# deepinv/deepinv

Measured on AMD Instinct MI355X. Metric: PnP-PGD slices/sec (50 iters), 2D MRI 8-coil 320x320, 4x radial mask, DRUNet, higher is better.
Workload: dtype f32: fp32 multiplies and accumulation on the fp32 matrix cores (v_mfma_f32_32x32x2_f32); ResBlock convs as Winograd F(4x4,3x3), U = G g G^T formed in fp64 and rounded once; the three 2x2 stride-2 down convolutions (2 % of the FLOPs) as an exact three-part bf16 operand split with six products and fp3

## Files before the change

### deepinv_amd/csrc/drunet_bf16s.hip

```cpp
#include "drunet_common.hpp"

using namespace dinv;
using namespace dinv_drunet;

namespace {

__device__ __forceinline__ unsigned f2bf(float f) {
#ifdef DINV_EMU
    unsigned u = __float_as_uint(f);
    if ((u & 0x7fffffffu) > 0x7f800000u) return (u >> 16) | 0x40u;
    u += 0x7fffu + ((u >> 16) & 1u);
    return u >> 16;
#else
    return (unsigned)__builtin_bit_cast(unsigned short, (__bf16)f);
#endif
}
__device__ __forceinline__ float bf2f(unsigned h) { return __uint_as_float(h << 16); }

__device__ __forceinline__ void split8(const float4& a, const float4& b, uint4& hi, uint4& lo) {
    const float v[8] = {a.x, a.y, a.z, a.w, b.x, b.y, b.z, b.w};
    unsigned h[8], l[8];
#pragma unroll
    for (int e = 0; e < 8; ++e) {
        h[e] = f2bf(v[e]);
        l[e] = f2bf(v[e] - bf2f(h[e]));
    }
    hi = make_uint4(h[0] | (h[1] << 16), h[2] | (h[3] << 16), h[4] | (h[5] << 16), h[6] | (h[7] << 16));
    lo = make_uint4(l[0] | (l[1] << 16), l[2] | (l[3] << 16), l[4] | (l[5] << 16), l[6] | (l[7] << 16));
}

__device__ __forceinline__ void split8x3(const float4& a, const float4& b, uint4& hi, uint4& mi, uint4& lo) {
    const float v[8] = {a.x, a.y, a.z, a.w, b.x, b.y, b.z, b.w};
    unsigned h[8], m[8], l[8];
#pragma unroll
    for (int e = 0; e < 8; ++e) {
        h[e] = f2bf(v[e]);
        const float r1 = v[e] - bf2f(h[e]);
        m[e] = f2bf(r1);
        l[e] = f2bf(r1 - bf2f(m[e]));
    }
    hi = make_uint4(h[0] | (h[1] << 16), h[2] | (h[3] << 16), h[4] | (h[5] << 16), h[6] | (h[7] << 16));
    mi = make_uint4(m[0] | (m[1] << 16), m[2] | (m[3] << 16), m[4] | (m[5] << 16), m[6] | (m[7] << 16));
    lo = make_uint4(l[0] | (l[1] << 16), l[2] | (l[3] << 16), l[4] | (l[5] << 16), l[6] | (l[7] << 16));
}

#ifdef DINV_EMU
__device__ __forceinline__ f32x16 mfma_bf16(const uint4& a, const uint4& b, const f32x16& c) {
    emu_bf16x8 av, bv;
    std::memcpy(&av, &a, 16);
    std::memcpy(&bv, &b, 16);
    return emu_mfma_f32_32x32x16_bf16(av, bv, c);
}
#else
typedef __bf16 bf16x8 __attribute__((ext_vector_type(8)));
__device__ __forceinline__ f32x16 mfma_bf16(const uint4& a, const uint4& b, const f32x16& c) {
    return __builtin_amdgcn_mfma_f32_32x32x16_bf16(__builtin_bit_cast(bf16x8, a), __builtin_bit_cast(bf16x8, b), c, 0, 0, 0);
}
#endif

struct DownSArgs {
    Geom gi, go;
    const float* x;
    const uint4* w;
    float* y;
    int32_t cin, cout;
    int64_t ntiles, per_xcd;
    DepthMap dm;
};

template <bool ACC, int NPL>
__global__ __launch_bounds__(256) void down2x2_bf16s_kernel(DownSArgs a) {
    constexpr int WU = NPL * 128;
    constexpr int WPT = (WU + 255) / 256;
    __shared__ uint4 wl[2][WU];
    const int tid = threadIdx.x, lane = tid & 63, wv = tid >> 6;
    const int l31 = lane & 31, lhi = lane >> 5;
    const int64_t logical = (int64_t)(blockIdx.x & 7) * a.per_xcd + (blockIdx.x >> 3);
    if (logical >= a.ntiles) return;
    const int nct = a.cout / 64;
    const int64_t q0 = (logical / nct) * 256 + wv * 64;
    const int co0 = (int)(logical % nct) * 64;
    int64_t ioff[2];
    bool in[2];
#pragma unroll
    for (int n = 0; n < 2; ++n) {
        const int64_t q = q0 + n * 32 + l31;
        in[n] = interior(a.go, q);
        ioff[n] = a.gi.sl;
        if (in[n]) {
            const int64_t b = q / a.go.plane;
            const int64_t bi = depth_pair(a.dm, b);
            if (bi < 0) in[n] = false;
            else {
                const int qi = (int)(q - b * a.go.plane);
                const int R = qi / a.go.wp, C = qi - R * a.go.wp;
                ioff[n] = a.gi.sl + bi * a.gi.plane + (int64_t)(2 * (R - 1) + 1) * a.gi.wp + (2 * (C - 1) + 1);
            }
        }
    }
    f32x16 acc[2][2];
#pragma unroll
    for (int m = 0; m < 2; ++m)
#pragma unroll
        for (int n = 0; n < 2; ++n)
#pragma unroll
            for (int r = 0; r < 16; ++r) acc[m][n][r] = 0.f;
    const int S = a.cin / 16, nsteps = 4 * S;
    float4 ba[2], bb[2];
    uint4 wreg[WPT];
    auto issue = [&](int g) {
        const int tap = g / S, s = g - tap * S;
        const int64_t toff = (int64_t)(tap >> 1) * a.gi.wp + (tap & 1);
#pragma unroll
        for (int k = 0; k < WPT; ++k) {
            const int u = tid + 256 * k;
            if (u < WU) wreg[k] = a.w[((int64_t)g * (2 * NPL) + (u >> 6)) * a.cout + co0 + (u & 63)];
        }
#pragma unroll
        for (int n = 0; n < 2; ++n) {
            const float* xb = a.x + ((int64_t)(2 * s + lhi) * a.gi.cs + ioff[n] + toff) * 8;
            ba[n] = ld4(xb);
            bb[n] = ld4(xb + 4);
        }
    };
    uint4 Bp[NPL][2];
    auto commit = [&](int stage) {
#pragma unroll
        for (int k = 0; k < WPT; ++k)
            if (tid + 256 * k < WU) wl[stage][tid + 256 * k] = wreg[k];
#pragma unroll
        for (int n = 0; n < 2; ++n) {
            if constexpr (NPL == 2) split8(ba[n], bb[n], Bp[0][n], Bp[1][n]);
            else split8x3(ba[n], bb[n], Bp[0][n], Bp[1][n], Bp[2][n]);
        }
    };
    issue(0);
    commit(0);
    if (nsteps > 1) issue(1);
    __syncthreads();
    constexpr int NPROD = NPL == 2 ? 3 : 6;
    constexpr int PA[6] = {0, 1, 0, 0, 1, 0}, PB2[3] = {1, 0, 0};
    constexpr int QA[6] = {1, 0, 2, 0, 1, 0}, QB[6] = {1, 2, 0, 1, 0, 0};
    for (int g = 0; g < nsteps; ++g) {
        const uint4* ws = wl[g & 1];
        uint4 A[NPL][2];
#pragma unroll
        for (int pl = 0; pl < NPL; ++pl)
#pragma unroll
            for (int m = 0; m < 2; ++m) A[pl][m] = ws[pl * 128 + lhi * 64 + m * 32 + l31];
#pragma unroll
        for (int e = 0; e < NPROD; ++e) {
            const int pa = NPL == 2 ? PA[e] : QA[e], pb = NPL == 2 ? PB2[e] : QB[e];
#pragma unroll
            for (int m = 0; m < 2; ++m)
#pragma unroll
                for (int n = 0; n < 2; ++n) acc[m][n] = mfma_bf16(A[pa][m], Bp[pb][n], acc[m][n]);
        }
        if (g + 1 < nsteps) {
            commit((g + 1) & 1);
            if (g + 2 < nsteps) issue(g + 2);
        }
        lds_barrier();
    }
#pragma unroll
    for (int n = 0; n < 2; ++n) {
        const int64_t q = q0 + n * 32 + l31;
        if (q >= a.go.np) continue;
        store_tile<2, false, ACC ? 1 : 0>(acc, n, a.go.sl + q, in[n], co0 / 8, a.cout / 8, a.go.cs, lhi, a.y, ACC ? a.y : nullptr,
                                          nullptr);
    }
}

struct UpSArgs {
    Geom gi, go;
    const float* x;
    const float* x2;
    const uint4* w;
    float* y;
    int32_t cin, cout;
    DepthMap dm;
};

#ifdef DINV_EMU
#define DINV_BF16S_UP_ATTR
#else
#define DINV_BF16S_UP_ATTR __attribute__((amdgpu_waves_per_eu(2, 2)))
#endif
template <bool SKIP>
__global__ __launch_bounds__(256) DINV_BF16S_UP_ATTR void up2x2_bf16s_kernel(UpSArgs a) {
    __shared__ uint4 wl[2][1024];
    const int tid = threadIdx.x, lane = tid & 63, wv = tid >> 6;
    const int l31 = lane & 31, lhi = lane >> 5;
    const int tp = wv & 1, pg = wv >> 1;
    const int co0 = blockIdx.y * 64;
    const int64_t p0 = (int64_t)blockIdx.x * 128 + pg * 64;
    int64_t ioff[2], ooff[2];
    bool in[2];
#pragma unroll
    for (int n = 0; n < 2; ++n) {
        const int64_t p = p0 + n * 32 + l31;
        in[n] = interior(a.gi, p);
        ioff[n] = a.gi.sl + (in[n] ? p : 0);
        ooff[n] = 0;
        if (in[n]) {
            const int64_t b = p / a.gi.plane;
            const int64_t bo = depth_pair(a.dm, b);
            if (bo < 0) in[n] = false;
            else {
                const int pi = (int)(p - b * a.gi.plane);
                const int r = pi / a.gi.wp, c = pi - r * a.gi.wp;
                ooff[n] = a.go.sl + bo * a.go.plane + (int64_t)(2 * (r - 1) + 1 + tp) * a.go.wp + (2 * (c - 1) + 1);
            }
        }
    }
    f32x16 acc[2][2][2];
#pragma unroll
    for (int t = 0; t < 2; ++t)
#pragma unroll
        for (int m = 0; m < 2; ++m)
#pragma unroll
            for (int n = 0; n < 2; ++n)
#pragma unroll
                for (int r = 0; r < 16; ++r) acc[t][m][n][r] = 0.f;
    const int S = a.cin / 16;
    float4 ba[2], bb[2];
    uint4 wreg[4];
    auto issue = [&](int s) {
#pragma unroll
        for (int k = 0; k < 4; ++k) {
            const int u = tid + 256 * k;
            wreg[k] = a.w[((int64_t)s * 16 + (u >> 6)) * a.cout + co0 + (u & 63)];
        }
#pragma unroll
        for (int n = 0; n < 2; ++n) {
            const int64_t o = ((int64_t)(2 * s + lhi) * a.gi.cs + ioff[n]) * 8;
            ba[n] = ld4(a.x + o);
            bb[n] = ld4(a.x + o + 4);
            if (SKIP) {
                ba[n] = add4(ba[n], ld4(a.x2 + o));
                bb[n] = add4(bb[n], ld4(a.x2 + o + 4));
            }
        }
    };
    auto commit = [&](int stage, uint4 (&Bh)[2], uint4 (&Bl)[2]) {
#pragma unroll
        for (int k = 0; k < 4; ++k) wl[stage][tid + 256 * k] = wreg[k];
        split8(ba[0], bb[0], Bh[0], Bl[0]);
        split8(ba[1], bb[1], Bh[1], Bl[1]);
    };
    uint4 Bh[2], Bl[2];
    issue(0);
    commit(0, Bh, Bl);
    if (S > 1) issue(1);
    __syncthreads();
    for (int s = 0; s < S; ++s) {
        const uint4* ws = wl[s & 1] + (tp * 2) * 256;
#pragma unroll
        for (int t = 0; t < 2; ++t) {
            uint4 A[2][2];
#pragma unroll
            for (int pl = 0; pl < 2; ++pl)
#pragma unroll
                for (int m = 0; m < 2; ++m) A[pl][m] = ws[t * 256 + pl * 128 + lhi * 64 + m * 32 + l31];
#pragma unroll
            for (int e = 0; e < 3; ++e) {
                const int pa = e == 1 ? 1 : 0;
#pragma unroll
                for (int m = 0; m < 2; ++m)
#pragma unroll
                    for (int n = 0; n < 2; ++n) acc[t][m][n] = mfma_bf16(A[pa][m], e == 0 ? Bl[n] : Bh[n], acc[t][m][n]);
            }
        }
        if (s + 1 < S) {
            commit((s + 1) & 1, Bh, Bl);
            if (s + 2 < S) issue(s + 2);
        }
        lds_barrier();
    }
#pragma unroll
    for (int n = 0; n < 2; ++n) {
        if (!in[n]) continue;
#pragma unroll
        for (int t = 0; t < 2; ++t)
#pragma unroll
            for (int m = 0; m < 2; ++m)
#pragma unroll
                for (int rj = 0; rj < 4; ++rj) {
                    const float4 v = make_float4(acc[t][m][n][4 * rj], acc[t][m][n][4 * rj + 1], acc[t][m][n][4 * rj + 2],
                                                 acc[t][m][n][4 * rj + 3]);
                    st4(a.y + ((int64_t)(co0 / 8 + m * 4 + rj) * a.go.cs + ooff[n] + t) * 8 + 4 * lhi, v);
                }
    }
}

}

static int down2x2_bf16s_launch(const dinv_act_geom* gin, const dinv_act_geom* gout, const float* x, const void* w_split,
                                int32_t cin, int32_t cout, float* y, DepthMap dm, int accumulate, dinv_stream_t stream,
                                int planes = 2) {
    if (int e = check_geom(gin)) return e;
    if (int e = check_geom(gout)) return e;
    DINV_REQUIRE(x && w_split && y, "null tensor pointer");
    DINV_REQUIRE(gin->height == 2 * gout->height && gin->width == 2 * gout->width, "down2x2 geometry mismatch");
    if (dm.dep_s == 0) DINV_REQUIRE(gin->batch == gout->batch, "down2x2 geometry mismatch");
    else
        DINV_REQUIRE(dm.dep_s >= 3 && dm.dep_l == 2 * (dm.dep_s - 2) + 2 && gout->batch % dm.dep_s == 0 &&
                     gin->batch / dm.dep_l == gout->batch / dm.dep_s && gin->batch % dm.dep_l == 0 && (dm.dz == 0 || dm.dz == 1),
                     "down2x2: bad depth pairing (%d, %d, %d)", dm.dep_s, dm.dep_l, dm.dz);
    DINV_REQUIRE(cin >= 16 && cin % 16 == 0 && cout % 64 == 0, "bf16-split down2x2 needs cin %% 16 == 0 and cout %% 64 == 0 (got %d,%d)", cin, cout);
    DownSArgs a{make_geom(*gin), make_geom(*gout), x, reinterpret_cast<const uint4*>(w_split), y, cin, cout, 0, 0, dm};
    a.ntiles = ceil_div(gout->np, 256) * (cout / 64);
    a.per_xcd = ceil_div(a.ntiles, 8);
    const dim3 grid((unsigned)(a.per_xcd * 8));
    hipStream_t st = reinterpret_cast<hipStream_t>(stream);
    if (planes == 3) hipLaunchKernelGGL((down2x2_bf16s_kernel<false, 3>), grid, dim3(256), 0, st, a);
    else if (accumulate) hipLaunchKernelGGL((down2x2_bf16s_kernel<true, 2>), grid, dim3(256), 0, st, a);
    else hipLaunchKernelGGL((down2x2_bf16s_kernel<false, 2>), grid, dim3(256), 0, st, a);
    DINV_CHECK_LAUNCH();
    return 0;
}

extern "C" int dinv_conv_down2x2_bf16s(const dinv_act_geom* gin, const dinv_act_geom* gout, const float* x,
                                       const void* w_split, int32_t cin, int32_t cout, float* y, dinv_stream_t stream) {
    return down2x2_bf16s_launch(gin, gout, x, w_split, cin, cout, y, DepthMap{0, 0, 0}, 0, stream);
}

extern "C" int dinv_conv_down2x2_bf16x3(const dinv_act_geom* gin, const dinv_act_geom* gout, const float* x,
                                        const void* w_split3, int32_t cin, int32_t cout, float* y, dinv_stream_t stream) {
    return down2x2_bf16s_launch(gin, gout, x, w_split3, cin, cout, y, DepthMap{0, 0, 0}, 0, stream, 3);
}

extern "C" int dinv_conv_down2x2_bf16s_3d(const dinv_act_geom* gin, const dinv_act_geom* gout, const float* x,
                                          const void* w_split, int32_t cin, int32_t cout, float* y, int32_t depth_out,
                                          int32_t dz, int32_t accumulate, dinv_stream_t stream) {
    DINV_REQUIRE(depth_out >= 1, "bad depth %d", depth_out);
    return down2x2_bf16s_launch(gin, gout, x, w_split, cin, cout, y, DepthMap{depth_out + 2, 2 * depth_out + 2, dz}, accumulate, stream);
}

static int up2x2_bf16s_launch(const dinv_act_geom* gin, const dinv_act_geom* gout, const float* x, const float* x2,
                              const void* w_split, int32_t cin, int32_t cout, float* y, DepthMap dm, dinv_stream_t stream) {
    if (int e = check_geom(gin)) return e;
    if (int e = check_geom(gout)) return e;
    DINV_REQUIRE(x && w_split && y, "null tensor pointer");
    DINV_REQUIRE(gout->height == 2 * gin->height && gout->width == 2 * gin->width, "up2x2 geometry mismatch");
    if (dm.dep_s == 0) DINV_REQUIRE(gin->batch == gout->batch, "up2x2 geometry mismatch");
    else
        DINV_REQUIRE(dm.dep_s >= 3 && dm.dep_l == 2 * (dm.dep_s - 2) + 2 && gin->batch % dm.dep_s == 0 &&
                     gout->batch % dm.dep_l == 0 && gout->batch / dm.dep_l == gin->batch / dm.dep_s && (dm.dz == 0 || dm.dz == 1),
                     "up2x2: bad depth pairing (%d, %d, %d)", dm.dep_s, dm.dep_l, dm.dz);
    DINV_REQUIRE(cin >= 16 && cin % 16 == 0 && cout % 64 == 0, "bf16-split up2x2 needs cin %% 16 == 0 and cout %% 64 == 0 (got %d,%d)", cin, cout);
    UpSArgs a{make_geom(*gin), make_geom(*gout), x, x2, reinterpret_cast<const uint4*>(w_split), y, cin, cout, dm};
    const dim3 grid((unsigned)ceil_div(gin->np, 128), (unsigned)(cout / 64));
    hipStream_t st = reinterpret_cast<hipStream_t>(stream);
    if (x2) hipLaunchKernelGGL(up2x2_bf16s_kernel<true>, grid, dim3(256), 0, st, a);
    else hipLaunchKernelGGL(up2x2_bf16s_kernel<false>, grid, dim3(256), 0, st, a);
    DINV_CHECK_LAUNCH();
    return 0;
}

extern "C" int dinv_conv_up2x2_bf16s(const dinv_act_geom* gin, const dinv_act_geom* gout, const float* x, const float* x2,
                                     const void* w_split, int32_t cin, int32_t cout, float* y, dinv_stream_t stream) {
    return up2x2_bf16s_launch(gin, gout, x, x2, w_split, cin, cout, y, DepthMap{0, 0, 0}, stream);
}

extern "C" int dinv_conv_up2x2_bf16s_3d(const dinv_act_geom* gin, const dinv_act_geom* gout, const float* x, const float* x2,
                                        const void* w_split, int32_t cin, int32_t cout, float* y, int32_t depth_in, int32_t dz,
                                        dinv_stream_t stream) {
    DINV_REQUIRE(depth_in >= 1, "bad depth %d", depth_in);
    return up2x2_bf16s_launch(gin, gout, x, x2, w_split, cin, cout, y, DepthMap{depth_in + 2, 2 * depth_in + 2, dz}, stream);
}
```

Before: 16.24.

## Deepen down2x2 bf16-split prefetch and add wide 128-channel output tile

Reworks the stride-2 down convolution kernel so each step keeps four register stages of weight and activation loads in flight, with the main loop unrolled by four. This hides global-load latency behind the MFMA work. Separately, it adds a wider tile variant covering 128 output channels per block, used only when enough tiles exist, so each activation split is reused across more MFMAs. The deeper prefetch costs more registers and issues redundant clamped loads near the end of the loop, and the wide path lowers the block count.

```diff
diff --git a/deepinv_amd/csrc/drunet_bf16s.hip b/deepinv_amd/csrc/drunet_bf16s.hip
--- a/deepinv_amd/csrc/drunet_bf16s.hip
+++ b/deepinv_amd/csrc/drunet_bf16s.hip
@@ -68,18 +68,20 @@
     DepthMap dm;
 };
 
-template <bool ACC, int NPL>
+template <bool ACC, int NPL, int MT>
 __global__ __launch_bounds__(256) void down2x2_bf16s_kernel(DownSArgs a) {
-    constexpr int WU = NPL * 128;
+    constexpr int CT = 32 * MT;
+    constexpr int WU = NPL * 2 * CT;
     constexpr int WPT = (WU + 255) / 256;
-    __shared__ uint4 wl[2][WU];
+    constexpr int PF = 4;
+    __shared__ uint4 wl[2][WPT * 256];
     const int tid = threadIdx.x, lane = tid & 63, wv = tid >> 6;
     const int l31 = lane & 31, lhi = lane >> 5;
     const int64_t logical = (int64_t)(blockIdx.x & 7) * a.per_xcd + (blockIdx.x >> 3);
     if (logical >= a.ntiles) return;
-    const int nct = a.cout / 64;
+    const int nct = a.cout / CT;
     const int64_t q0 = (logical / nct) * 256 + wv * 64;
-    const int co0 = (int)(logical % nct) * 64;
+    const int co0 = (int)(logical % nct) * CT;
     int64_t ioff[2];
     bool in[2];
 #pragma unroll
@@ -98,75 +100,85 @@
             }
         }
     }
-    f32x16 acc[2][2];
-#pragma unroll
-    for (int m = 0; m < 2; ++m)
+    f32x16 acc[MT][2];
+#pragma unroll
+    for (int m = 0; m < MT; ++m)
 #pragma unroll
         for (int n = 0; n < 2; ++n)
 #pragma unroll
             for (int r = 0; r < 16; ++r) acc[m][n][r] = 0.f;
     const int S = a.cin / 16, nsteps = 4 * S;
-    float4 ba[2], bb[2];
-    uint4 wreg[WPT];
-    auto issue = [&](int g) {
+    struct Raw {
+        float4 ba[2], bb[2];
+        uint4 w[WPT];
+    };
+    auto issue = [&](Raw& r, int g) {
+        g = min(g, nsteps - 1);
         const int tap = g / S, s = g - tap * S;
         const int64_t toff = (int64_t)(tap >> 1) * a.gi.wp + (tap & 1);
 #pragma unroll
         for (int k = 0; k < WPT; ++k) {
-            const int u = tid + 256 * k;
-            if (u < WU) wreg[k] = a.w[((int64_t)g * (2 * NPL) + (u >> 6)) * a.cout + co0 + (u & 63)];
+            const int u = tid + 256 * k < WU ? tid + 256 * k : tid;
+            r.w[k] = a.w[((int64_t)g * (2 * NPL) + u / CT) * a.cout + co0 + u % CT];
         }
 #pragma unroll
         for (int n = 0; n < 2; ++n) {
             const float* xb = a.x + ((int64_t)(2 * s + lhi) * a.gi.cs + ioff[n] + toff) * 8;
-            ba[n] = ld4(xb);
-            bb[n] = ld4(xb + 4);
+            r.ba[n] = ld4(xb);
+            r.bb[n] = ld4(xb + 4);
         }
     };
     uint4 Bp[NPL][2];
-    auto commit = [&](int stage) {
-#pragma unroll
-        for (int k = 0; k < WPT; ++k)
-            if (tid + 256 * k < WU) wl[stage][tid + 256 * k] = wreg[k];
+    auto commit = [&](const Raw& r, int stage) {
+#pragma unroll
+        for (int k = 0; k < WPT; ++k) wl[stage][tid + 256 * k] = r.w[k];
 #pragma unroll
         for (int n = 0; n < 2; ++n) {
-            if constexpr (NPL == 2) split8(ba[n], bb[n], Bp[0][n], Bp[1][n]);
-            else split8x3(ba[n], bb[n], Bp[0][n], Bp[1][n], Bp[2][n]);
-        }
-    };
-    issue(0);
-    commit(0);
-    if (nsteps > 1) issue(1);
-    __syncthreads();
+            if constexpr (NPL == 2) split8(r.ba[n], r.bb[n], Bp[0][n], Bp[1][n]);
+            else split8x3(r.ba[n], r.bb[n], Bp[0][n], Bp[1][n], Bp[2][n]);
+        }
+    };
     constexpr int NPROD = NPL == 2 ? 3 : 6;
     constexpr int PA[6] = {0, 1, 0, 0, 1, 0}, PB2[3] = {1, 0, 0};
     constexpr int QA[6] = {1, 0, 2, 0, 1, 0}, QB[6] = {1, 2, 0, 1, 0, 0};
-    for (int g = 0; g < nsteps; ++g) {
-        const uint4* ws = wl[g & 1];
-        uint4 A[NPL][2];
+    auto step = [&](int g, int stage, Raw& next) {
+        const uint4* ws = wl[stage];
+        uint4 A[NPL][MT];
 #pragma unroll
         for (int pl = 0; pl < NPL; ++pl)
 #pragma unroll
-            for (int m = 0; m < 2; ++m) A[pl][m] = ws[pl * 128 + lhi * 64 + m * 32 + l31];
+            for (int m = 0; m < MT; ++m) A[pl][m] = ws[(pl * 2 + lhi) * CT + m * 32 + l31];
 #pragma unroll
         for (int e = 0; e < NPROD; ++e) {
             const int pa = NPL == 2 ? PA[e] : QA[e], pb = NPL == 2 ? PB2[e] : QB[e];
 #pragma unroll
-            for (int m = 0; m < 2; ++m)
+            for (int m = 0; m < MT; ++m)
 #pragma unroll
                 for (int n = 0; n < 2; ++n) acc[m][n] = mfma_bf16(A[pa][m], Bp[pb][n], acc[m][n]);
         }
-        if (g + 1 < nsteps) {
-            commit((g + 1) & 1);
-            if (g + 2 < nsteps) issue(g + 2);
-        }
+        commit(next, stage ^ 1);
+        issue(next, g + 1 + PF);
         lds_barrier();
+    };
+    Raw r0, r1, r2, r3;
+    issue(r0, 0);
+    issue(r1, 1);
+    issue(r2, 2);
+    issue(r3, 3);
+    commit(r0, 0);
+    issue(r0, PF);
+    __syncthreads();
+    for (int g = 0; g < nsteps; g += PF) {
+        step(g, 0, r1);
+        step(g + 1, 1, r2);
+        step(g + 2, 0, r3);
+        step(g + 3, 1, r0);
     }
 #pragma unroll
     for (int n = 0; n < 2; ++n) {
         const int64_t q = q0 + n * 32 + l31;
         if (q >= a.go.np) continue;
-        store_tile<2, false, ACC ? 1 : 0>(acc, n, a.go.sl + q, in[n], co0 / 8, a.cout / 8, a.go.cs, lhi, a.y, ACC ? a.y : nullptr,
+        store_tile<MT, false, ACC ? 1 : 0>(acc, n, a.go.sl + q, in[n], co0 / 8, a.cout / 8, a.go.cs, lhi, a.y, ACC ? a.y : nullptr,
                                           nullptr);
     }
 }
@@ -295,6 +307,11 @@
 
 }
 
+#ifndef DINV_DOWN_WIDE_MIN
+#define DINV_DOWN_WIDE_MIN 512
+#endif
+constexpr int64_t DOWN_WIDE_MIN = DINV_DOWN_WIDE_MIN;
+
 static int down2x2_bf16s_launch(const dinv_act_geom* gin, const dinv_act_geom* gout, const float* x, const void* w_split,
                                 int32_t cin, int32_t cout, float* y, DepthMap dm, int accumulate, dinv_stream_t stream,
                                 int planes = 2) {
@@ -309,13 +326,19 @@
                      "down2x2: bad depth pairing (%d, %d, %d)", dm.dep_s, dm.dep_l, dm.dz);
     DINV_REQUIRE(cin >= 16 && cin % 16 == 0 && cout % 64 == 0, "bf16-split down2x2 needs cin %% 16 == 0 and cout %% 64 == 0 (got %d,%d)", cin, cout);
     DownSArgs a{make_geom(*gin), make_geom(*gout), x, reinterpret_cast<const uint4*>(w_split), y, cin, cout, 0, 0, dm};
-    a.ntiles = ceil_div(gout->np, 256) * (cout / 64);
+    const int64_t wide_tiles = ceil_div(gout->np, 256) * (cout / 128);
+    const bool wide = cout % 128 == 0 && wide_tiles >= DOWN_WIDE_MIN;
+    a.ntiles = wide ? wide_tiles : ceil_div(gout->np, 256) * (cout / 64);
     a.per_xcd = ceil_div(a.ntiles, 8);
     const dim3 grid((unsigned)(a.per_xcd * 8));
     hipStream_t st = reinterpret_cast<hipStream_t>(stream);
-    if (planes == 3) hipLaunchKernelGGL((down2x2_bf16s_kernel<false, 3>), grid, dim3(256), 0, st, a);
-    else if (accumulate) hipLaunchKernelGGL((down2x2_bf16s_kernel<true, 2>), grid, dim3(256), 0, st, a);
-    else hipLaunchKernelGGL((down2x2_bf16s_kernel<false, 2>), grid, dim3(256), 0, st, a);
+#define DINV_DOWN_LAUNCH(ACC, NPL)                                                                                      \
+    if (wide) hipLaunchKernelGGL((down2x2_bf16s_kernel<ACC, NPL, 4>), grid, dim3(256), 0, st, a);                       \
+    else hipLaunchKernelGGL((down2x2_bf16s_kernel<ACC, NPL, 2>), grid, dim3(256), 0, st, a)
+    if (planes == 3) { DINV_DOWN_LAUNCH(false, 3); }
+    else if (accumulate) { DINV_DOWN_LAUNCH(true, 2); }
+    else { DINV_DOWN_LAUNCH(false, 2); }
+#undef DINV_DOWN_LAUNCH
     DINV_CHECK_LAUNCH();
     return 0;
 }
```

Result: no change. 16.35 (median of 6 runs) (+0.7%).
